# voletiv/mcvd-pytorch

Hardware: AMD Instinct MI355X
Metric: sampled frames/sec (whole node), SMMNIST 64x64 DDPM 100-step (higher is better)
Workload: dtype f32-equivalent: f32 storage and accumulation; 58 of 58 3x3 convs, 41 of 41 1x1 convs and the attention products (head dims 32..128) as SIX bf16 piece products of operands split EXACTLY into three bf16 pieces (all 24 bits, fp32 exponent range, less than one fp32 rounding per product; tests/test_gpu_p

## Files before the change

### mcvd_pytorch_amd/csrc/api.cpp

```cpp
#include <dlfcn.h>
#include <errno.h>
#include <fcntl.h>
#include <pthread.h>
#include <math.h>
#include <sys/file.h>
#include <sys/stat.h>
#include <unistd.h>
#include <stdio.h>
#include <stdlib.h>
#include <string.h>

#include <algorithm>
#include <cmath>
#include <mutex>
#include <new>
#include <vector>

#include "model.h"
#include "conv_kernels.h"
#include "inception.h"
#include "lpips.h"

using namespace mcvd;

// ... 298 lines not shown
    if (ok) { ctx->wino_selftest = 1; return 0; }
    ctx->wino_selftest = -1;
    ctx->bf16x3 = 0;
    ++ctx->epoch;
    set_error("self-test of the hand-scheduled Winograd kernels FAILED on this device (kernels that ran: %d %d %d; |bf16x3 - fp32 MFMA| = %.3e at "
              "scale %.3e; %zu values of the persistent form differ from the per-item form): the option bf16x3 was switched off for this context",
              ran[0], ran[1], ran[2], (double)d10, (double)scale, diff16);
    return MCVD_ESELFTEST;
    API_CATCH
}

int mcvd_ctx_clear_range(mcvd_ctx* ctx) {
    API_TRY
    MCVD_REQUIRE(ctx, "ctx is NULL");
    if (ctx->range_flag) MCVD_HIP_CHECK(hipMemsetAsync(ctx->range_flag, 0, sizeof(int), ctx->stream));
    return 0;
    API_CATCH
}

int mcvd_ctx_set_option(mcvd_ctx* ctx, const char* key, int value) {
    MCVD_REQUIRE(ctx && key, "ctx/key is NULL");
    ++ctx->epoch;
    if (!strcmp(key, "naive_conv")) ctx->naive_conv = value;
    else if (!strcmp(key, "naive_attn")) ctx->naive_attn = value;
    else if (!strcmp(key, "fir_form")) ctx->fir_form = value;
    else if (!strcmp(key, "dbg_skip_finalize")) ctx->dbg_skip_finalize = value;
    else if (!strcmp(key, "gn_producer")) ctx->gn_producer = value;
    else if (!strcmp(key, "graph")) ctx->graph = value;
    else if (!strcmp(key, "conv_shape")) ctx->conv_shape = value;
    else if (!strcmp(key, "conv_shape1")) ctx->conv_shape1 = value;
    else if (!strcmp(key, "profile")) ctx->profile = value;
    else if (!strcmp(key, "conv_wdma")) ctx->conv_wdma = value;
    else if (!strcmp(key, "autotune")) ctx->autotune = value;
    else if (!strcmp(key, "side_stream")) ctx->side_stream = value;
    else if (!strcmp(key, "share_fence")) ctx->share_fence = value;
    else if (!strcmp(key, "winograd")) ctx->winograd = value;
    else if (!strcmp(key, "conv_dma1")) ctx->conv_dma1 = value;
    else if (!strcmp(key, "bf16x3")) ctx->bf16x3 = value;
    else if (!strcmp(key, "f16x2")) {
        if (ctx->f16x2 != value) (void)mcvd_ctx_clear_range(ctx);
        ctx->f16x2 = value;
    }
    else if (!strcmp(key, "f16x1")) {
        if (ctx->f16x1 != value) (void)mcvd_ctx_clear_range(ctx);
        ctx->f16x1 = value;
    }
    else if (!strcmp(key, "conv_cot")) ctx->conv_cot = value;
    else if (!strcmp(key, "persist_grid")) ctx->persist_grid = value;
    else if (!strcmp(key, "temb_table")) ctx->temb_table = value;
    else if (!strcmp(key, "im2col_lds")) ctx->im2col_lds = value;
    else if (!strcmp(key, "gn_stats")) ctx->gn_stats = value;
    else if (!strcmp(key, "spade_fuse")) ctx->spade_fuse = value;
    else if (!strcmp(key, "attn_presplit")) ctx->attn_presplit = value;
    else {
        set_error("unknown option '%s'", key);
        return MCVD_EINVAL;
    }
    return 0;
}

static void default_schedule(mcvd_model* m) {
    const int T = m->d.num_classes;
    m->betas.assign(T, 0.f);
    m->alphas.assign(T, 0.f);
    m->alphas_prev.assign(T, 0.f);
    if (m->d.sigma_dist == 0) {
        const float start = m->d.sigma_begin, end = m->d.sigma_end;
        const float step = (end - start) / (float)(T - 1);
        for (int i = 0; i < T; ++i) m->betas[i] = (i < T / 2) ? start + step * (float)i : end - step * (float)(T - 1 - i);
        float p = 1.0f;
        for (int i = T - 1; i >= 0; --i) {
            p = p * (1.0f - m->betas[i]);
            m->alphas[i] = p;
        }
        for (int i = 0; i < T; ++i) m->alphas_prev[i] = (i + 1 < T) ? m->alphas[i + 1] : 1.0f;
    } else {
        std::vector<float> f(T + 1);
        const float s = 0.008f;
        for (int i = 0; i <= T; ++i) {
            const float t = (float)(T - i) / (float)T;
            const float c = cosf((t + s) / (1.0f + s) * (float)(M_PI / 2));
            f[i] = c * c;
        }
        for (int i = 0; i < T; ++i) m->alphas[i] = f[i] / f[T];
        for (int i = 0; i < T; ++i) m->alphas_prev[i] = (i + 1 < T) ? m->alphas[i + 1] : 1.0f;
        for (int i = 0; i < T; ++i) m->betas[i] = 1.0f - m->alphas[i] / m->alphas_prev[i];
    }
    const int half = m->d.ngf / 2;
    m->freqs.assign(half, 0.f);
    const float e = (float)(-(log(10000.0) / (double)(half - 1)));
    for (int k = 0; k < half; ++k) m->freqs[k] = expf((float)k * e);
}

int mcvd_model_create(mcvd_ctx* ctx, const mcvd_unet_desc* desc, mcvd_model** out) {
    API_TRY
    MCVD_REQUIRE(desc && out, "model_create: NULL argument");
    MCVD_REQUIRE(desc->sigma_dist == 0 || desc->sigma_dist == 1, "desc: sigma_dist=%d", desc->sigma_dist);
    mcvd_model* m = new mcvd_model();
    m->ctx = ctx;
    m->d = *desc;
    if (m->build_plan()) {
        delete m;
        return MCVD_EINVAL;
    }
    default_schedule(m);
    if (ctx) {
// ... 351 lines not shown
        kinds[i] = (int)op.kind;
        ks[i] = op.kind == OP_CONV ? op.ks : 0;
        ms[i] = t;
        const double HW = (double)op.H * op.W;
        const double cin = op.src0.C + (op.src1.kind == REF_NONE ? 0 : op.src1.C);
        double f = 0, by = 0;
        switch (op.kind) {
            case OP_CONV:
                f = 2.0 * B * HW * op.Cout * cin * op.ks * op.ks;
                by = 4.0 * (B * HW * (cin + op.Cout + (op.res.kind != REF_NONE ? op.Cout : 0)) + cin * op.ks * op.ks * op.Cout);
                break;
            case OP_GN: by = 4.0 * B * HW * cin; f = 4.0 * B * HW * cin; break;
            case OP_FIR: {
                const double o = op.up ? 4.0 : 0.25;
                by = 4.0 * B * HW * op.src0.C * (1.0 + o * (op.dst2.kind != REF_NONE ? 2.0 : 1.0));
                f = B * HW * op.src0.C * o * (op.up ? 8.0 : 32.0);
                break;
            }
            case OP_ATTN:
                f = 4.0 * B * HW * HW * op.Cout;
                by = 4.0 * B * HW * op.Cout * 4.0;
                break;
            case OP_APPLY: by = 4.0 * B * HW * cin * 4.0; f = 12.0 * B * HW * cin; break;
            case OP_TEMB: f = 2.0 * B * (m->d.ngf * m->T + (double)m->T * m->T); by = 4.0 * (m->d.ngf * m->T + (double)m->T * m->T); break;
            case OP_DENSE: f = 2.0 * B * m->T * m->NE; by = 4.0 * ((double)m->T * m->NE + B * m->NE); break;
            default: break;
        }
        flops[i] = f;
        bytes[i] = by;
    }
    return n;
}

int mcvd_model_op_info(mcvd_model* m, int i, int info[8]) {
    MCVD_REQUIRE(m && info && i >= 0 && i < (int)m->ops.size(), "op_info: index %d", i);
    const Op& op = m->ops[i];
    info[0] = (int)op.kind; info[1] = op.module; info[2] = op.ks; info[3] = op.H;
    info[4] = op.src0.C + (op.src1.kind == REF_NONE ? 0 : op.src1.C); info[5] = op.Cout;
    info[6] = op.res.kind != REF_NONE; info[7] = op.coef.kind != REF_NONE;
    if ((size_t)i < m->tuned_shape.size() && m->tuned_shape[i] >= 0) info[6] |= (m->tuned_shape[i] << 4) | (m->tuned_cot[i] << 8) | (1 << 12);
    return 0;
}

int mcvd_model_op_kernel(mcvd_model* m, int i) {
    if (!m || i < 0 || i >= (int)m->ops.size() || m->ops[i].kind != OP_CONV || (size_t)i >= m->ran_kernel.size()) return -1;
    return m->ran_kernel[i];
}

int mcvd_model_op_attention_kernel(mcvd_model* m, int i) {
    if (!m || i < 0 || i >= (int)m->ops.size() || m->ops[i].kind != OP_ATTN || (size_t)i >= m->ran_attn.size()) return -1;
    return m->ran_attn[i];
}

long mcvd_model_fused_launches(mcvd_model* m, int what) { return (m && what >= 0 && what < 4) ? m->fused_launches[what] : -1; }

int mcvd_model_module_output(mcvd_model* m, int module, int B, float* dst, int64_t capacity, int* C, int* H) {
    MCVD_REQUIRE(m && dst && B > 0 && B <= m->arena_B, "module_output: run a forward at batch >= B first");
    const Op* last = nullptr;
    for (const Op& op : m->ops)
        if (op.module == module && op.dst.kind == REF_ARENA) last = &op;
    MCVD_REQUIRE(last, "module_output: module %d has no workspace output", module);
    const int c = last->dst.C;
    int h = last->H;
    if (last->kind == OP_FIR) h = last->up ? 2 * h : h / 2;
    if (last->kind == OP_TEMB || last->kind == OP_DENSE) h = 0;
    const int64_t per = h ? (int64_t)c * h * h : c;
    MCVD_REQUIRE(per * B <= capacity, "module_output: capacity %lld < %lld", (long long)capacity, (long long)(per * B));
    MCVD_HIP_CHECK(hipMemcpyAsync(dst, m->arena + last->dst.off * (int64_t)B, (size_t)per * B * sizeof(float),
                                  hipMemcpyDeviceToDevice, m->ctx->stream));
    if (C) *C = c;
    if (H) *H = h;
    return 0;
}

struct GuidedCall {
    const float* cond_weak;
    float w;
    int weak_mask;
};

static int guided_begin(mcvd_model* m, const char* who, const float* cond, const GuidedCall& g, int B) {
    MCVD_REQUIRE(m->d.num_frames_cond > 0 && cond, "%s: guidance needs a net with conditioning frames (and its cond)", who);
    MCVD_REQUIRE(!m->d.noise_in_cond, "%s: guidance on a noise_in_cond net is not defined (two z per evaluation)", who);
    MCVD_REQUIRE(B <= (1 << 29), "%s: B = %d", who, B);
    if (int rc = m->prepare_B(2 * B)) return rc;
    if (int rc = m->ensure_guided(B, g.weak_mask)) return rc;
    const size_t cbytes = (size_t)B * m->d.channels * m->d.num_frames_cond * m->d.image_size * m->d.image_size * sizeof(float);
    hipStream_t s = m->ctx->stream;
    MCVD_HIP_CHECK(hipMemcpyAsync(m->gd_cond, cond, cbytes, hipMemcpyDeviceToDevice, s));
    char* weak = reinterpret_cast<char*>(m->gd_cond) + cbytes;
    if (g.cond_weak) MCVD_HIP_CHECK(hipMemcpyAsync(weak, g.cond_weak, cbytes, hipMemcpyDeviceToDevice, s));
    else MCVD_HIP_CHECK(hipMemsetAsync(weak, 0, cbytes, s));
    m->cond_cache_valid = false;
    return 0;
}

static int guided_dup_x(mcvd_model* m, const float* x, int64_t n) {
    hipStream_t s = m->ctx->stream;
    MCVD_HIP_CHECK(hipMemcpyAsync(m->gd_x, x, (size_t)n * sizeof(float), hipMemcpyDeviceToDevice, s));
    MCVD_HIP_CHECK(hipMemcpyAsync(m->gd_x + n, x, (size_t)n * sizeof(float), hipMemcpyDeviceToDevice, s));
    return 0;
}

static int sampler_run_impl(mcvd_model* m, int kind, float* x, const float* cond, const float* noise, uint64_t seed,
                            uint64_t sample_offset, int subsample_steps, int flags, double t_min, int B, const GuidedCall* g) {
    MCVD_REQUIRE(m && x && B > 0, "sampler_run: bad arguments");
    MCVD_REQUIRE(kind == MCVD_SAMPLER_DDPM || kind == MCVD_SAMPLER_DDIM, "sampler_run: kind %d", kind);
// ... 772 lines not shown
```

### mcvd_pytorch_amd/csrc/common.h

```cpp
#pragma once
#include <hip/hip_runtime.h>
#include <stdint.h>
#include <atomic>
#include <string>

#include "conv_kernels.h"


namespace mcvd {

__device__ __forceinline__ float fma_unpacked(float x, float a, float b) {
    float r;
    asm("v_fma_f32 %0, %1, %2, %3" : "=v"(r) : "v"(x), "v"(a), "v"(b));
    return r;
}

void set_error(const char* fmt, ...);
const char* get_error();

#define MCVD_HIP_CHECK(expr)                                                                  \
    do {                                                                                      \
        hipError_t _e = (expr);                                                               \
        if (_e != hipSuccess) {                                                               \
            mcvd::set_error("%s failed: %s (%s:%d)", #expr, hipGetErrorString(_e), __FILE__, __LINE__); \
// ... 15 lines not shown
        int dev = 0;
        if (hipGetDevice(&dev) != hipSuccess || dev < 0 || dev >= 64) return true;
        const unsigned long long bit = 1ull << dev;
        return (mask.load(std::memory_order_acquire) & bit) == 0;
    }
    void done() {
        int dev = 0;
        if (hipGetDevice(&dev) == hipSuccess && dev >= 0 && dev < 64) mask.fetch_or(1ull << dev, std::memory_order_release);
    }
};

static inline int ceil_div(int a, int b) { return (a + b - 1) / b; }
static inline int round_up(int a, int b) { return ceil_div(a, b) * b; }

struct GnOut {
    float* coef;
    int groups;
    float eps;
    int mode;
    const float* p0;
    const float* p1;
    int emb_stride, emb_off;
};

struct ConvArgs {
    const float* x0;
    const float* x1;
    int C0, C1;
    const float* coef;
    int act;
    const float* wp;
    const float* wpw;
    const float* wph;
    const float* wpb;
    const float* bias;
    const float* res;
    float out_scale;
    float* y;
    int B, Cin, CinP, Cout, CoutP, H, W;
    int ks;
    int cot;
    int shape_hint;
    int ksplit;
    float* part;
    size_t part_floats;
    int wdma;
    int pgrid;
    unsigned long long* dbg;
    float* stats;
    const float* gb;
    const float* coef2;
    float* kv_img;
    int kv_C, kv_D;
    int im2col;
    GnOut gno;
};
int last_conv_gn_fused();
void set_last_conv_gn_fused(int v);
bool ksplit_reduce_gn_usable(const ConvArgs& a);
int launch_ksplit_reduce_gn(const ConvArgs& a, hipStream_t s);
bool conv1x1_h2_kv_supported(const ConvArgs& a, int cot);
void set_last_conv_stats_np(int np);
int last_conv_stats_np();
int conv_cout_tile(int Cout);
int conv_chunk(int ks);
int launch_conv_mfma(const ConvArgs& a, hipStream_t s);
int launch_conv_naive(const ConvArgs& a, hipStream_t s);
int last_conv_kernel();
bool conv_kernel_usable(int id, const ConvArgs& a);
int conv_kernel_launch(int id, const ConvArgs& a, hipStream_t s);
int launch_im2col3x3(const float* x0, int C0, const float* x1, int C1, float* col, int B, int H, int W, int K, hipStream_t s);
int launch_taps_shift_add(const float* z, const float* bias, const float* res, float scale, float* y, int B, int Cout, int H, int W, hipStream_t s);
int launch_pack_conv_gemm_form(const float* w, float* wp, int Cout, int Cin, int form, int CoutP, hipStream_t s);
int conv_wino_require(ConvFamily family, const ConvArgs& a, const char* what);
dim3 wino_grid(const ConvArgs& a, bool g8, int bco, int parts);
int wino_launch_done(const ConvArgs& a, bool g8, int parts, hipStream_t s);
bool conv_wino_supported(int ks, int H, int W);
int conv_wino_cout_tile(int Cout);
int launch_conv_wino(const ConvArgs& a, hipStream_t s);
int launch_wino_ksplit_reduce(const ConvArgs& a, hipStream_t s);
int launch_conv_wino3(const ConvArgs& a, hipStream_t s);
long conv_wino3_weight_floats(int CinP, int CoutP);
int launch_conv_wino3p(const ConvArgs& a, hipStream_t s);
int launch_pack_wino3_weight(const float* w, float* wb, int Cout, int Cin, int CinP, int CoutP, hipStream_t s);
int launch_conv_wino2h(const ConvArgs& a, int np, hipStream_t s);
long conv_wino2h_weight_floats(int CinP, int CoutP);
int launch_pack_wino2h_weight(const float* w, float* wh, int Cout, int Cin, int CinP, int CoutP, hipStream_t s);
bool conv1x1_h2_supported(const ConvArgs& a, int cot, int np);
int launch_conv1x1_h2(const ConvArgs& a, int cot, hipStream_t s, int np);
long conv1x1_h2_weight_floats(int CinP, int CoutP, int np);
int launch_pack_conv1x1_h2(const float* wp, float* wh, int CinP, int CoutP, hipStream_t s, int np);
bool conv1x1_dma_supported(const ConvArgs& a, int ck, int pxw = 1);
int conv1x1_dma_cout_tile(int CoutP);
int launch_conv1x1_dma(const ConvArgs& a, int cot_req, int ck, hipStream_t s, int pxw = 1);
int launch_pack_wino_weight(const float* w, float* up, int Cout, int Cin, int CinP, int CoutP, hipStream_t s);
int launch_pack_conv_weight(const float* w, float* wp, int Cout, int Cin, int ks, int CinP, int CoutP, int nin,
                            int cout_off, hipStream_t s);

struct GnArgs {
    const float* x0;
    const float* x1;
    int C0, C1;
    int groups;
    float eps;
    int mode;
    const float* p0;
    const float* p1;
    int emb_stride, emb_off;
    float* coef;
    int B, HW;
};
int launch_gn_coef(const GnArgs& a, hipStream_t s);
int launch_gn_finalize(const GnArgs& a, const float* st0, int np0, const float* st1, int np1, hipStream_t s);

// ... 83 lines not shown
```

### mcvd_pytorch_amd/csrc/kernels/conv1x1_h2.cpp

```cpp
#include <stdlib.h>

#include "../common.h"
#include "pieces.h"

namespace mcvd {

typedef float f32x16 __attribute__((ext_vector_type(16)));
typedef float f32x2 __attribute__((ext_vector_type(2)));
typedef unsigned u32x4 __attribute__((ext_vector_type(4)));

__device__ __forceinline__ float silu_q(float v) { return v * __builtin_amdgcn_rcpf(1.0f + __expf(-v)); }

constexpr int Q1_PT = 128;
constexpr int Q1_CK = 16;
constexpr int Q1_NB = 4;
constexpr int Q1_MAXIMG = 4;

template <int NP, int COT, int PRO, int EXP = 0, bool KV = false, bool IM = false>
__global__ __launch_bounds__(256, 2) void conv1x1_h2_kernel(ConvArgs a, int ptiles, int nct) {
    typedef Pieces<NP> PX;
    constexpr int PT = Q1_PT, CK = Q1_CK, NB = Q1_NB, BCO = 32 * COT;
    constexpr int PPR = PT / 4;
    constexpr int RPS = 256 / PPR;
    constexpr int XSZ = CK * PT;
// ... 432 lines not shown
        if constexpr (NP == 3)
            MCVD_HIP_CHECK(hipFuncSetAttribute(reinterpret_cast<const void*>(&conv1x1_h2_kernel<3, COT, 1, 0, true>), hipFuncAttributeMaxDynamicSharedMemorySize, 160 * 1024));
        raised.done();
    }
#ifdef MCVD_DIAG
    {
        const char* es = getenv("MCVD_Q1_EXP");
        const int e = es ? atoi(es) : 0;
        if (e != 0 && NP == 3 && COT == 3) {
            static PerDeviceOnce raised2;
            if (raised2.first_use()) {
                (void)hipFuncSetAttribute(reinterpret_cast<const void*>(&conv1x1_h2_kernel<3, 3, 1, 1>), hipFuncAttributeMaxDynamicSharedMemorySize, 160 * 1024);
                (void)hipFuncSetAttribute(reinterpret_cast<const void*>(&conv1x1_h2_kernel<3, 3, 1, 2>), hipFuncAttributeMaxDynamicSharedMemorySize, 160 * 1024);
                (void)hipFuncSetAttribute(reinterpret_cast<const void*>(&conv1x1_h2_kernel<3, 3, 1, 4>), hipFuncAttributeMaxDynamicSharedMemorySize, 160 * 1024);
                (void)hipFuncSetAttribute(reinterpret_cast<const void*>(&conv1x1_h2_kernel<3, 3, 1, 6>), hipFuncAttributeMaxDynamicSharedMemorySize, 160 * 1024);
                (void)hipFuncSetAttribute(reinterpret_cast<const void*>(&conv1x1_h2_kernel<3, 3, 1, 7>), hipFuncAttributeMaxDynamicSharedMemorySize, 160 * 1024);
                (void)hipFuncSetAttribute(reinterpret_cast<const void*>(&conv1x1_h2_kernel<3, 3, 1, 15>), hipFuncAttributeMaxDynamicSharedMemorySize, 160 * 1024);
                (void)hipFuncSetAttribute(reinterpret_cast<const void*>(&conv1x1_h2_kernel<3, 3, 1, 16>), hipFuncAttributeMaxDynamicSharedMemorySize, 160 * 1024);
                raised2.done();
            }
            switch (e) {
                case 1: hipLaunchKernelGGL((conv1x1_h2_kernel<3, 3, 1, 1>), grid, dim3(256), lds, s, a, ptiles, nct); break;
                case 2: hipLaunchKernelGGL((conv1x1_h2_kernel<3, 3, 1, 2>), grid, dim3(256), lds, s, a, ptiles, nct); break;
                case 4: hipLaunchKernelGGL((conv1x1_h2_kernel<3, 3, 1, 4>), grid, dim3(256), lds, s, a, ptiles, nct); break;
                case 6: hipLaunchKernelGGL((conv1x1_h2_kernel<3, 3, 1, 6>), grid, dim3(256), lds, s, a, ptiles, nct); break;
                case 7: hipLaunchKernelGGL((conv1x1_h2_kernel<3, 3, 1, 7>), grid, dim3(256), lds, s, a, ptiles, nct); break;
                case 16: hipLaunchKernelGGL((conv1x1_h2_kernel<3, 3, 1, 16>), grid, dim3(256), lds, s, a, ptiles, nct); break;
                default: hipLaunchKernelGGL((conv1x1_h2_kernel<3, 3, 1, 15>), grid, dim3(256), lds, s, a, ptiles, nct); break;
            }
            MCVD_HIP_CHECK(hipGetLastError());
            return 0;
        }
    }
    if constexpr (NP == 3) {
        static const bool noprio = getenv("MCVD_Q1_NOPRIO") && atoi(getenv("MCVD_Q1_NOPRIO")) != 0;
        if (noprio) {
            static PerDeviceOnce raised3;
            if (raised3.first_use()) {
                (void)hipFuncSetAttribute(reinterpret_cast<const void*>(&conv1x1_h2_kernel<NP, COT, 0, 16>), hipFuncAttributeMaxDynamicSharedMemorySize, 160 * 1024);
                (void)hipFuncSetAttribute(reinterpret_cast<const void*>(&conv1x1_h2_kernel<NP, COT, 1, 16>), hipFuncAttributeMaxDynamicSharedMemorySize, 160 * 1024);
                (void)hipFuncSetAttribute(reinterpret_cast<const void*>(&conv1x1_h2_kernel<NP, COT, 2, 16>), hipFuncAttributeMaxDynamicSharedMemorySize, 160 * 1024);
                raised3.done();
            }
            if (!a.coef) hipLaunchKernelGGL((conv1x1_h2_kernel<NP, COT, 0, 16>), grid, dim3(256), lds, s, a, ptiles, nct);
            else if (!a.act) hipLaunchKernelGGL((conv1x1_h2_kernel<NP, COT, 1, 16>), grid, dim3(256), lds, s, a, ptiles, nct);
            else hipLaunchKernelGGL((conv1x1_h2_kernel<NP, COT, 2, 16>), grid, dim3(256), lds, s, a, ptiles, nct);
            MCVD_HIP_CHECK(hipGetLastError());
            return 0;
        }
    }
#endif
    if constexpr (NP == 3) {
        if (a.kv_img && a.coef && !a.act) {
            hipLaunchKernelGGL((conv1x1_h2_kernel<3, COT, 1, 0, true>), grid, dim3(256), lds, s, a, ptiles, nct);
            MCVD_HIP_CHECK(hipGetLastError());
            return 0;
        }
    }
    if (!a.coef)
        hipLaunchKernelGGL((conv1x1_h2_kernel<NP, COT, 0>), grid, dim3(256), lds, s, a, ptiles, nct);
    else if (!a.act)
        hipLaunchKernelGGL((conv1x1_h2_kernel<NP, COT, 1>), grid, dim3(256), lds, s, a, ptiles, nct);
    else
        hipLaunchKernelGGL((conv1x1_h2_kernel<NP, COT, 2>), grid, dim3(256), lds, s, a, ptiles, nct);
    MCVD_HIP_CHECK(hipGetLastError());
    return 0;
}

template <int NP>
static int q1_launch_cot(const ConvArgs& a, int cot, hipStream_t s) {
    switch (cot) {
        case 1: return q1_launch<NP, 1>(a, s);
        case 2: return q1_launch<NP, 2>(a, s);
        case 3: return q1_launch<NP, 3>(a, s);
        default: return q1_launch<NP, 4>(a, s);
    }
}

bool conv1x1_h2_kv_supported(const ConvArgs& a, int cot) {
    return a.kv_img && a.kv_C > 0 && a.Cout == 3 * a.kv_C && a.kv_D % 32 == 0 && a.kv_C % a.kv_D == 0 && a.coef && !a.act && !a.res && a.out_scale == 1.0f &&
           !a.stats && conv1x1_h2_supported(a, cot, 3);
}

int launch_conv1x1_h2(const ConvArgs& a, int cot, hipStream_t s, int np) {
    MCVD_REQUIRE(!a.kv_img || (np == 3 && conv1x1_h2_kv_supported(a, cot)), "conv1x1 split-operand GEMM: K / V piece images requested for a launch that cannot write them");
    MCVD_REQUIRE(conv1x1_h2_supported(a, cot, np), "conv1x1 split-operand GEMM: unsupported (np=%d ks=%d H=%d W=%d Cin=%d C0=%d cot=%d, weight pieces %s)",
                 np, a.ks, a.H, a.W, a.Cin, a.C0, cot, (np == 2 ? a.wph : a.wpb) ? "present" : "missing");
    const int rc = np == 2 ? q1_launch_cot<2>(a, cot, s) : q1_launch_cot<3>(a, cot, s);
    const int HW = a.H * a.W;
    if (rc == 0 && a.stats && (HW >= Q1_PT || HW == 64)) set_last_conv_stats_np(HW >= Q1_PT ? HW / Q1_PT : 1);
    return rc;
}

__global__ void q1_absmax_kernel(const float* w, long n, unsigned* hdr) {
    float m = 0.0f;
    for (long i = blockIdx.x * (long)blockDim.x + threadIdx.x; i < n; i += (long)gridDim.x * blockDim.x) m = fmaxf(m, fabsf(w[i]));
#pragma unroll
    for (int o = 32; o > 0; o >>= 1) m = fmaxf(m, __shfl_xor(m, o));
    if ((threadIdx.x & 63) == 0) atomicMax(hdr, __float_as_uint(m));
}

__global__ void pack_conv1x1_h2_kernel(const float* wp, float* wh, int CinP, int CoutP) {
    const float wmax = wh[0];
    int k = 0;
    (void)frexpf(wmax, &k);
    const int e = (wmax > 0.0f && wmax < 3.0e38f) ? min(max(14 - k, -60), 60) : 0;
    const float scale = ldexpf(1.0f, e);
    if (blockIdx.x == 0 && threadIdx.x == 0) { wh[1] = scale; wh[2] = ldexpf(1.0f, -e); }
    _Float16* dst = reinterpret_cast<_Float16*>(wh + Pieces<2>::HDR);
    const long n = (long)CinP * CoutP;
    const int NS = CoutP / 32;
    for (long i = blockIdx.x * (long)blockDim.x + threadIdx.x; i < n; i += (long)gridDim.x * blockDim.x) {
        const int co = (int)(i % CoutP), ci = (int)(i / CoutP);
        const float us = wp[i] * scale;
        const _Float16 h1 = (_Float16)us;
        const _Float16 h2 = (_Float16)(us - (float)h1);
        const int cc = ci & 15, h = cc & 1, el = cc >> 1, lane = h * 32 + (co & 31);
        const long o = (((long)(ci >> 4) * NS + (co >> 5)) * 2) * 512 + (lane * 4 + (el >> 1)) * 2 + (el & 1);
        dst[o] = h1;
        dst[o + 512] = h2;
    }
}

__global__ void pack_conv1x1_b3_kernel(const float* wp, unsigned short* dst, int CinP, int CoutP) {
    const long n = (long)CinP * CoutP;
    const int NS = CoutP / 32;
    for (long i = blockIdx.x * (long)blockDim.x + threadIdx.x; i < n; i += (long)gridDim.x * blockDim.x) {
        const int co = (int)(i % CoutP), ci = (int)(i / CoutP);
        const float u = wp[i];
        const unsigned short h1 = px_bf16_rne(u);
        const float r1 = u - px_bf16_f32(h1);
        const unsigned short h2 = px_bf16_rne(r1);
        const float r2 = r1 - px_bf16_f32(h2);
        const unsigned short h3 = px_bf16_rne(r2);
        const int cc = ci & 15, h = cc & 1, el = cc >> 1, lane = h * 32 + (co & 31);
        const long o = (((long)(ci >> 4) * NS + (co >> 5)) * 3) * 512 + (lane * 4 + (el >> 1)) * 2 + (el & 1);
        dst[o] = h1;
        dst[o + 512] = h2;
        dst[o + 1024] = h3;
    }
// ... 22 lines not shown
```

### mcvd_pytorch_amd/csrc/model.cpp

```cpp
#include "model.h"
#include "conv_kernels.h"

#include <math.h>
#include <stdarg.h>
#include <stdio.h>
#include <string.h>

#include <algorithm>
#include <tuple>

namespace mcvd {

static thread_local char g_err[1024] = "";
void set_error(const char* fmt, ...) {
    va_list ap;
    va_start(ap, fmt);
    vsnprintf(g_err, sizeof(g_err), fmt, ap);
    va_end(ap);
}
const char* get_error() { return g_err; }

static int gn_groups(int ch) {
    int g = std::min(ch / 4, 32);
    while (g > 1 && ch % g != 0) --g;
// ... 749 lines not shown
        const int np = pieces(a.shape_hint);
        for (int c = 4; c >= 1 && !conv1x1_h2_supported(a, a.cot, np); --c)
            if (conv1x1_h2_supported(a, c, np)) a.cot = c;
    }
    if (!(a.shape_hint < 0 && tuned_B == a.B && oi < tuned_shape.size() && tuned_shape[oi] >= 0)) return;
    a.shape_hint = tuned_shape[oi];
    a.cot = tuned_cot[oi];
    const bool raw_in = conv_input_raw(op);
    if (!ctx->f16x1 || raw_in) a.shape_hint = without_f16x1(a.shape_hint);
    if ((!ctx->f16x2 || raw_in) && without_f16x2(a.shape_hint) != a.shape_hint) {
        a.shape_hint = without_f16x2(a.shape_hint);
        if (conv_kernel(a.shape_hint).own_cot && !conv_kernel_usable(a.shape_hint, a)) a.cot = op.cot;
    }
    if (!ctx->bf16x3 && without_bf16x3(a.shape_hint) != a.shape_hint) {
        a.shape_hint = without_bf16x3(a.shape_hint);
        a.cot = op.cot;
    }
}

int mcvd_model::apply_spade(const Op& op, const Io& io, ConvArgs& a) {
    if (a.shape_hint == CK_RETIRED_SPADE_WINO || a.shape_hint == CK_RETIRED_SPADE_WINO_K2) a.shape_hint = CK_AUTO;
    const bool want_fused = ctx->spade_fuse && !ctx->naive_conv && ctx->winograd;
    ConvArgs t = a;
    t.shape_hint = a.shape_hint == CK_WINO_K2 ? CK_WINO_K2 : CK_WINO;
    t.ksplit = k_parts(t.shape_hint);
    bool fused = want_fused && conv_kernel_usable(CK_WINO, t);
    if (!fused && t.ksplit == 2) { t.ksplit = 0; t.shape_hint = CK_WINO; fused = want_fused && conv_kernel_usable(CK_WINO, t); }
    if (fused) {
        a.shape_hint = t.shape_hint;
        ++fused_launches[2];
        return 0;
    }
    float* tmp = resolve(op.tmp, io);
    if (int rc = launch_spade_apply(a.x0, a.C0, a.x1, a.C1, a.coef, a.gb, a.coef2, tmp, a.B, op.H * op.W, op_stream ? op_stream : ctx->stream)) return rc;
    read_materialised(a, tmp);
    return 0;
}

void mcvd_model::set_gn_producer(const Op& op, const Io& io, ConvArgs& a) {
    gn_done[op.gn_next] = 0;
    if (ctx->gn_producer && ctx->gn_stats && a.stats && op.ks == 3 && !ctx->dbg_skip_finalize) gn_params(a.gno, ops[op.gn_next], io);
}

void mcvd_model::set_kv_presplit(const Op& op, const Io& io, ConvArgs& a) {
    kv_live[op.attn_op] = 0;
    const Op& at = ops[op.attn_op];
    const bool want = ctx->attn_presplit && !ctx->naive_conv && ctx->bf16x3 && !ctx->f16x2 && (ctx->naive_attn == 0 || ctx->naive_attn == 4) &&
                      !(ctx->share_fence && mcvd_ctx_shares_device(ctx)) && attn_h2p_supported(at.Cout, at.heads, at.H * at.W) && a.shape_hint == CK_GEMM1_BF16X3;
    if (!want) return;
    ConvArgs t = a;
    t.kv_img = resolve(op.kv, io);
    t.kv_C = at.Cout;
    t.kv_D = at.Cout / at.heads;
    if (conv1x1_h2_kv_supported(t, t.cot)) {
        a = t;
        kv_live[op.attn_op] = 1;
    }
}

int mcvd_model::launch_conv_op(const Op& op, const Io& io) {
    hipStream_t s = op_stream ? op_stream : ctx->stream;
    const size_t oi = (size_t)(&op - ops.data());
    ConvArgs a = conv_args(op, io, true);
    MCVD_REQUIRE(a.x0 && (a.C1 == 0 || a.x1), "forward: module %d needs a conditioning tensor (cond is NULL)", op.module);
    select_hint(op, a);
    if (op.gb.kind != REF_NONE)
        if (int rc = apply_spade(op, io, a)) return rc;
    a.stats = (ctx->gn_stats && op.stats.kind != REF_NONE && !ctx->naive_conv && (op.ks == 3 || ctx->gn_stats >= 2 || conv_kernel(a.shape_hint).family == CF_SPLIT1))
                  ? resolve(op.stats, io) : nullptr;
    if (ran_kernel.size() != ops.size()) ran_kernel.assign(ops.size(), -1);
    if (kv_live.size() != ops.size()) kv_live.assign(ops.size(), 0);
    if (gn_done.size() != ops.size()) gn_done.assign(ops.size(), 0);
    if (op.gn_next >= 0) set_gn_producer(op, io, a);
    if (op.attn_op >= 0) set_kv_presplit(op, io, a);
    if (ctx->naive_conv) {
        stats_np[oi] = 0;
        ran_kernel[oi] = -2;
        return launch_conv_naive(a, s);
    }
    if (conv_kernel(a.shape_hint).family == CF_GEMM3) {
        if (gemm_form_usable(op, a)) {
            const int rc = launch_gemm_form(op, a, resolve(op.alt_buf, io), s);
            stats_np[oi] = a.stats ? last_conv_stats_np() : 0;
            ran_kernel[oi] = op.alt_kind;
            return rc;
        }
        a.shape_hint = CK_AUTO;
        a.cot = op.cot;
    }
    const int rc = launch_conv_mfma(a, s);
    stats_np[oi] = a.stats ? last_conv_stats_np() : 0;
    ran_kernel[oi] = last_conv_kernel();
    if (rc == 0 && a.gno.coef && last_conv_gn_fused()) {
        gn_done[op.gn_next] = 1;
        ++fused_launches[3];
    }
    return rc;
}

int mcvd_model::launch_op(const Op& op, const float* x, const void* lab, const float* cond, float* out, int B) {
    hipStream_t s = op_stream ? op_stream : ctx->stream;
    const Io io{x, cond, out, B};
    auto at = [&](const TRef& r) { return resolve(r, io); };
    switch (op.kind) {
        case OP_TEMB: {
            if (temb_row_live) return 0;
            const float* w0 = blob + params[find_param("unet.all_modules.0.weight")].off;
            const float* b0 = blob + params[find_param("unet.all_modules.0.bias")].off;
            const float* w1 = blob + params[find_param("unet.all_modules.1.weight")].off;
            const float* b1 = blob + params[find_param("unet.all_modules.1.bias")].off;
            const float* emb = d.cond_emb ? blob + params[find_param("unet.all_modules.2.weight")].off : nullptr;
            return launch_temb_mlp(lab, labels_f32, packed + freqs_off, w0, b0, w1, b1, at(op.dst), one_temb_row() ? 1 : B, d.ngf, T, emb, cond_mask, s);
        }
        case OP_DENSE:
            if (temb_row_live) return 0;
            return launch_dense_all(at(op.src0), packed + dense_wt, packed + dense_bias, at(op.dst), one_temb_row() ? 1 : B, T, NE, s);
        case OP_GN:
            return launch_gn(op, io);
        case OP_CONV:
            return launch_conv_op(op, io);
        case OP_FIR: {
            const float* gb = at(op.gb);
            return launch_fir2(at(op.src0), at(op.coef), op.act, op.up, at(op.dst), B, op.src0.C, op.H, op.W, gb,
                               gb ? gb + (size_t)op.src0.C * op.H * op.W : nullptr, at(op.coef2), at(op.dst2), s, ctx->fir_form);
        }
        case OP_NEAREST:
            MCVD_REQUIRE(cond, "forward: SPADE model needs the conditioning tensor");
            return launch_nearest_resize(at(op.src0), at(op.dst), B * op.src0.C, d.image_size, d.image_size, op.H, op.W, s);
        case OP_CONDNOISE: {
            MCVD_REQUIRE(cond, "forward: noise_in_cond model needs the conditioning tensor");
            MCVD_REQUIRE(!labels_f32, "forward: noise_in_cond indexes alphas with the labels; float timesteps are not valid there");
            const int64_t per = (int64_t)op.src0.C * d.image_size * d.image_size;
            if (!alphas_dev) MCVD_HIP_CHECK(hipMalloc((void**)&alphas_dev, (size_t)d.num_classes * sizeof(float)));
            if (!alphas_dev_valid) {
                MCVD_HIP_CHECK(hipMemcpyAsync(alphas_dev, alphas.data(), (size_t)d.num_classes * sizeof(float), hipMemcpyHostToDevice, s));
                alphas_dev_valid = true;
            }
            const float* z = cond_noise_src;
            if (z) {
                cond_noise_src += per * B;
            } else {
                if (cond_gamma_k > 0.0f) {
                    if (int rc = launch_gamma_noise(cond_z, nullptr, cond_gamma_k, cond_gamma_theta, cond_gamma_kt, cond_gamma_sd,
                                                    cond_noise_seed, cond_noise_offset, (1ull << 32) + cond_noise_draw, B, per, s))
                        return rc;
// ... 366 lines not shown
```

### mcvd_pytorch_amd/csrc/model.h

```cpp
#pragma once
#include <atomic>
#include <map>
#include <string>
#include <vector>

#include "../../include/mcvd_hip.h"
#include "common.h"
#include "conv_tuner.h"

struct mcvd_ctx {
    int device = 0;
    int shared_device = 0;
    hipStream_t stream = nullptr;
    int naive_conv = 0;
    int naive_attn = 0;
    int gn_producer = 1;
    int dbg_skip_finalize = 0;
    int fir_form = 0;
    int graph = 0;
    hipStream_t cap = nullptr;
    std::atomic<unsigned> epoch{0};
    int conv_shape = -1;
    int conv_shape1 = -1;
    int winograd = 1;
    int persist_grid = 0;
    int temb_table = 1;
    int im2col_lds = 1;
    int wino_selftest = 0;
    int conv_cot = 0;
    int bf16x3 = 1;
    int f16x2 = 0;
    int f16x1 = 0;
    int conv_dma1 = 1;
    int conv_wdma = 1;
    int share_fence = 0;
    int side_stream = 0;
    hipStream_t side = nullptr;
    hipEvent_t ev_fork = nullptr, ev_join = nullptr;
    int spade_fuse = 0;
    int attn_presplit = 1;
    int gn_stats = 1;
    int autotune = 1;
    int profile = 0;
    unsigned long long* dbg = nullptr;
    const float* spade_gb = nullptr;
    const float* spade_coef2 = nullptr;
    float* stats_buf = nullptr;
    int* range_flag = nullptr;
    float* scratch = nullptr;
    size_t scratch_bytes = 0;
    int ensure_scratch(size_t bytes);
};

bool mcvd_ctx_shares_device(const mcvd_ctx* c);

namespace mcvd {

struct ParamInfo {
    std::string name;
    int64_t shape[4] = {0, 0, 0, 0};
    int ndim = 0;
    int64_t off = 0;
    int64_t numel = 0;
    bool set = false;
};

enum RefKind { REF_NONE = 0, REF_ARENA, REF_X, REF_COND, REF_OUT };
struct TRef {
    RefKind kind = REF_NONE;
    int64_t off = 0;
    int C = 0;
};

enum OpKind { OP_TEMB, OP_DENSE, OP_GN, OP_CONV, OP_FIR, OP_ATTN, OP_NEAREST, OP_COEF2, OP_APPLY, OP_CONDNOISE };

struct Op {
    OpKind kind;
    int module = -1;
    TRef src0, src1, dst, res;
    int H = 0, W = 0;
    int Cout = 0, ks = 0;
    int groups = 0;
    float eps = 0.f;
    int gn_mode = 0;
    int64_t p0 = -1, p1 = -1;
    int emb_off = 0;
    TRef coef;
    int act = 0;
    int64_t wp = -1, bias = -1;
    int64_t wpw = -1;
    int64_t wph = -1;
    int64_t wpb = -1;
    int CinP = 0, CoutP = 0, cot = 0;
// ... 54 lines not shown
    float* blob = nullptr;

    std::vector<mcvd::Op> ops;
    std::vector<mcvd::DenseEntry> dense;
    std::vector<mcvd::ConvPack> packs;
    int64_t packed_floats = 0;
    float* packed = nullptr;
    long long* coef2_desc_dev = nullptr;
    int coef2_first = -1, coef2_count = 0, coef2_cmax = 0;
    float* packed_h = nullptr;
    int64_t packed_h_floats = 0;
    bool packed_h_valid = false;
    int ensure_f16x2_weights();
    int64_t dense_wt = -1, dense_bias = -1, freqs_off = -1;
    int NE = 0;
    int T = 0;
    int first_module = 2;
    mcvd::TRef cond_src;
    const int32_t* cond_mask = nullptr;
    float* alphas_dev = nullptr;
    bool alphas_dev_valid = false;
    float* cond_z = nullptr;
    const float* cond_noise_src = nullptr;
    uint64_t cond_noise_seed = 0, cond_noise_offset = 0, cond_noise_draw = 0;
    float cond_gamma_kt = 0.f, cond_gamma_sd = 1.f;
    float* noise_buf = nullptr;
    float cond_gamma_k = 0.f, cond_gamma_theta = 0.f;
    std::vector<float> k_cum, theta_t;
    float* gamma_dev = nullptr;
    bool gamma_dev_valid = false;
    float* dsm_buf = nullptr;
    int dsm_B = 0;

    int64_t arena_per_sample = 0;
    float* arena = nullptr;
    int arena_B = 0;
    int64_t* labels = nullptr;
    float* eps_buf = nullptr;
    float* labels_f = nullptr;
    float* fp_buf = nullptr;
    int fp_B = 0;
    float* gd_x = nullptr;
    float* gd_cond = nullptr;
    int32_t* gd_mask = nullptr;
    int gd_B = 0, gd_mask_B = 0, gd_mask_val = -1;
    int ensure_guided(int B, int weak_mask);
    float* ksplit_buf = nullptr;
    size_t ksplit_floats = 0;

    std::vector<float> betas, alphas, alphas_prev, freqs;

    std::vector<int> stats_np;
    std::vector<signed char> kv_live;
    long fused_launches[4] = {0, 0, 0, 0};
    std::vector<signed char> gn_done;
    std::vector<int> ran_kernel;
    std::vector<int> ran_attn;
    std::vector<int> tuned_shape, tuned_cot;
    int tuned_B = 0;
    int tuned_sig = -1;
    std::map<int, std::pair<std::vector<int>, std::vector<int>>> tuned_cache;
    int autotune(int B);
    void sync_tuning_options();
    mcvd::TunerOptions tuner_options() const;
    mcvd::TunerLayer tuner_layer(const mcvd::Op& op, int B) const;

    std::vector<hipEvent_t> ev;
    bool profile_armed = false;
    int profile_B = 0;

    const float* prepared_cond = nullptr;
    int prepared_B = 0;
    bool cond_cache_valid = false;
    bool has_prep = false;
    int prepare_B(int B);
    int run_prep(const float* cond, int B);
    int prepare_cond(const float* cond, int B);

    struct GraphKey {
        const float* x = nullptr; const void* lab = nullptr; const float* cond = nullptr; float* out = nullptr;
        const void* mask = nullptr;
        int B = 0, labels_f32 = 0; unsigned epoch = 0, ctx_epoch = 0;
        bool operator==(const GraphKey& o) const {
            return x == o.x && lab == o.lab && cond == o.cond && out == o.out && mask == o.mask && B == o.B &&
                   labels_f32 == o.labels_f32 && epoch == o.epoch && ctx_epoch == o.ctx_epoch;
        }
    };
    GraphKey graph_key, graph_seen;
    hipGraphExec_t graph_exec = nullptr;
    unsigned epoch = 0;
    long graph_replays = 0, graph_captures = 0;
    void drop_graph();
    int forward_ops(const float* x, const void* labels, const float* cond, float* out, int B);

    hipStream_t op_stream = nullptr;
    int build_plan();
    int add_param(const std::string& name, std::initializer_list<int64_t> shape);
    int find_param(const char* name) const;
    int ensure_workspace(int B);
    int ensure_ksplit(int B);
    float* temb_tab = nullptr;
    float* temb_tmp = nullptr;
    int64_t* temb_lab = nullptr;
    size_t temb_rows_cap = 0;
    int temb_row_live = 0;
    int profile_temb_skipped = 0;
    int prepare_temb_table(const std::vector<int>& labels);
// ... 22 lines not shown
```

Before: 260.5.

## Add pixel-stationary split-operand QKV 1x1 conv kernel with LDS-resident activation pieces

Adds a new kernel for the attention q|k|v 1x1 projection. Each block splits a 64-pixel activation tile (with the per-channel affine coefficient applied) into bf16 pieces once and keeps them in LDS. Waves then stream weight pieces for many 32-channel output slices against that tile, writing Q directly and K/V as presplit piece images. The intent is to stop re-reading and re-splitting activations for every output tile, and the new path is on by default through a new option. The cost is a large dynamic LDS allocation (up to 160KB), which limits occupancy, and a grid-sizing heuristic tuned to 256 CUs.

```diff
diff --git a/mcvd_pytorch_amd/csrc/api.cpp b/mcvd_pytorch_amd/csrc/api.cpp
--- a/mcvd_pytorch_amd/csrc/api.cpp
+++ b/mcvd_pytorch_amd/csrc/api.cpp
@@ -374,6 +374,7 @@
     else if (!strcmp(key, "gn_stats")) ctx->gn_stats = value;
     else if (!strcmp(key, "spade_fuse")) ctx->spade_fuse = value;
     else if (!strcmp(key, "attn_presplit")) ctx->attn_presplit = value;
+    else if (!strcmp(key, "qkv_stationary")) ctx->qkv_stationary = value;
     else {
         set_error("unknown option '%s'", key);
         return MCVD_EINVAL;
@@ -831,7 +832,7 @@
     return m->ran_attn[i];
 }
 
-long mcvd_model_fused_launches(mcvd_model* m, int what) { return (m && what >= 0 && what < 4) ? m->fused_launches[what] : -1; }
+long mcvd_model_fused_launches(mcvd_model* m, int what) { return (m && what >= 0 && what < 5) ? m->fused_launches[what] : -1; }
 
 int mcvd_model_module_output(mcvd_model* m, int module, int B, float* dst, int64_t capacity, int* C, int* H) {
     MCVD_REQUIRE(m && dst && B > 0 && B <= m->arena_B, "module_output: run a forward at batch >= B first");
diff --git a/mcvd_pytorch_amd/csrc/common.h b/mcvd_pytorch_amd/csrc/common.h
--- a/mcvd_pytorch_amd/csrc/common.h
+++ b/mcvd_pytorch_amd/csrc/common.h
@@ -91,6 +91,7 @@
     const float* coef2;
     float* kv_img;
     int kv_C, kv_D;
+    int kv_stationary;
     int im2col;
     GnOut gno;
 };
@@ -99,6 +100,10 @@
 bool ksplit_reduce_gn_usable(const ConvArgs& a);
 int launch_ksplit_reduce_gn(const ConvArgs& a, hipStream_t s);
 bool conv1x1_h2_kv_supported(const ConvArgs& a, int cot);
+bool conv1x1_h2s_admits(const ConvArgs& a);
+int launch_conv1x1_h2s(const ConvArgs& a, hipStream_t s);
+int last_conv_qkv_stationary();
+void set_last_conv_qkv_stationary(int v);
 void set_last_conv_stats_np(int np);
 int last_conv_stats_np();
 int conv_cout_tile(int Cout);
diff --git a/mcvd_pytorch_amd/csrc/kernels/conv1x1_h2.cpp b/mcvd_pytorch_amd/csrc/kernels/conv1x1_h2.cpp
--- a/mcvd_pytorch_amd/csrc/kernels/conv1x1_h2.cpp
+++ b/mcvd_pytorch_amd/csrc/kernels/conv1x1_h2.cpp
@@ -508,6 +508,10 @@
 #endif
     if constexpr (NP == 3) {
         if (a.kv_img && a.coef && !a.act) {
+            if (a.kv_stationary && conv1x1_h2s_admits(a)) {
+                set_last_conv_qkv_stationary(1);
+                return launch_conv1x1_h2s(a, s);
+            }
             hipLaunchKernelGGL((conv1x1_h2_kernel<3, COT, 1, 0, true>), grid, dim3(256), lds, s, a, ptiles, nct);
             MCVD_HIP_CHECK(hipGetLastError());
             return 0;
@@ -542,6 +546,7 @@
     MCVD_REQUIRE(!a.kv_img || (np == 3 && conv1x1_h2_kv_supported(a, cot)), "conv1x1 split-operand GEMM: K / V piece images requested for a launch that cannot write them");
     MCVD_REQUIRE(conv1x1_h2_supported(a, cot, np), "conv1x1 split-operand GEMM: unsupported (np=%d ks=%d H=%d W=%d Cin=%d C0=%d cot=%d, weight pieces %s)",
                  np, a.ks, a.H, a.W, a.Cin, a.C0, cot, (np == 2 ? a.wph : a.wpb) ? "present" : "missing");
+    set_last_conv_qkv_stationary(0);
     const int rc = np == 2 ? q1_launch_cot<2>(a, cot, s) : q1_launch_cot<3>(a, cot, s);
     const int HW = a.H * a.W;
     if (rc == 0 && a.stats && (HW >= Q1_PT || HW == 64)) set_last_conv_stats_np(HW >= Q1_PT ? HW / Q1_PT : 1);
diff --git a/mcvd_pytorch_amd/csrc/kernels/conv1x1_h2s.cpp b/mcvd_pytorch_amd/csrc/kernels/conv1x1_h2s.cpp
--- /dev/null
+++ b/mcvd_pytorch_amd/csrc/kernels/conv1x1_h2s.cpp
@@ -0,0 +1,232 @@
+#include "../common.h"
+#include "pieces.h"
+
+namespace mcvd {
+
+typedef float f32x16 __attribute__((ext_vector_type(16)));
+typedef float f32x4 __attribute__((ext_vector_type(4)));
+typedef float f32x2 __attribute__((ext_vector_type(2)));
+typedef unsigned u32x4 __attribute__((ext_vector_type(4)));
+
+constexpr int S1_PT = 64;
+constexpr int S1_CK = 16;
+constexpr int S1_WAVES = 8;
+constexpr int S1_PITCH = 36;
+constexpr int S1_SLICE = 32 * S1_PITCH;
+constexpr int S1_CUS = 256;
+constexpr size_t S1_LDS_MAX = 160 * 1024;
+
+static size_t s1_lds_bytes(int Cin) { return (size_t)Cin * (S1_PT * 3 * 2) + (size_t)S1_WAVES * S1_SLICE * sizeof(float); }
+
+__global__ __launch_bounds__(S1_WAVES * 64) void conv1x1_h2s_kernel(ConvArgs a, int tiles, int ng, int upg, int nunits) {
+    typedef Pieces<3> PX;
+    extern __shared__ __attribute__((aligned(16))) float smem[];
+    const int tid = threadIdx.x, lane = tid & 63, l31 = lane & 31, half = lane >> 5;
+    const int wave = __builtin_amdgcn_readfirstlane(tid >> 6);
+    const int Cin = a.Cin, nchunks = Cin / S1_CK, HW = a.H * a.W, NS = a.CoutP / 32;
+    u32x4* sB = reinterpret_cast<u32x4*>(smem);
+    float* sO = smem + nchunks * (2 * 3 * 256) + wave * S1_SLICE;
+
+    int tile, grp;
+    if (tiles < 8) {
+        tile = blockIdx.x % tiles;
+        grp = blockIdx.x / tiles;
+    } else {
+        const int xcd = blockIdx.x & 7, slot = blockIdx.x >> 3;
+        tile = (slot / ng) * 8 + xcd;
+        grp = slot - (slot / ng) * ng;
+    }
+    if (tile >= tiles || grp >= ng) return;
+    const int b = (int)(((long)tile * S1_PT) / HW), p0 = (int)((long)tile * S1_PT - (long)b * HW);
+
+    {
+        const float* xb = a.x0 + (long)b * a.C0 * HW + p0 + l31;
+        const float* cb = a.coef + (long)b * Cin * 2;
+        const int nitems = nchunks * 2;
+        for (int it = wave; it < nitems; it += 2 * S1_WAVES) {
+            float bv[2][8];
+            f32x2 cf[2][8];
+#pragma unroll
+            for (int u = 0; u < 2; ++u) {
+                const int item = it + u * S1_WAVES;
+                if (item < nitems) {
+                    const int c0 = (item >> 1) * S1_CK + half;
+                    const float* xs = xb + (long)c0 * HW + (item & 1) * 32;
+#pragma unroll
+                    for (int e = 0; e < 8; ++e) {
+                        bv[u][e] = xs[(long)(2 * e) * HW];
+                        cf[u][e] = *reinterpret_cast<const f32x2*>(cb + (c0 + 2 * e) * 2);
+                    }
+                }
+            }
+#pragma unroll
+            for (int u = 0; u < 2; ++u) {
+                const int item = it + u * S1_WAVES;
+                if (item < nitems) {
+#pragma unroll
+                    for (int e = 0; e < 8; ++e)
+                        asm("v_fma_f32 %0, %1, %2, %3" : "=v"(bv[u][e]) : "v"(bv[u][e]), "v"(cf[u][e].x), "v"(cf[u][e].y));
+                    unsigned w[4][3];
+#pragma unroll
+                    for (int j = 0; j < 4; ++j) PX::split<false>(bv[u][2 * j], bv[u][2 * j + 1], w[j]);
+#pragma unroll
+                    for (int p = 0; p < 3; ++p) sB[(item * 3 + p) * 64 + lane] = u32x4{w[0][p], w[1][p], w[2][p], w[3][p]};
+                }
+            }
+        }
+    }
+    __syncthreads();
+
+    const int lo = grp * upg, hi = min(lo + upg, nunits);
+    const u32x4* wq = reinterpret_cast<const u32x4*>(a.wpb) + lane;
+    const int Cq = a.kv_C, D = a.kv_D, DT = D >> 5, heads = Cq / D, ntl = HW >> 5;
+    unsigned* img = reinterpret_cast<unsigned*>(a.kv_img);
+#define S1_LOADA(SET, st, c)                                                        \
+    {                                                                               \
+        const u32x4* w_ = wq + ((long)(c) * NS + (st)) * (3 * 64);                  \
+        SET[0] = w_[0]; SET[1] = w_[64]; SET[2] = w_[128];                          \
+    }
+#define S1_READB(SET, c)                                                            \
+    {                                                                               \
+        const u32x4* b_ = sB + (c) * (2 * 3 * 64) + lane;                           \
+        _Pragma("unroll") for (int q = 0; q < 6; ++q) SET[q] = b_[q * 64];          \
+    }
+#define S1_MMA(AC, BC)                                                              \
+    _Pragma("unroll") for (int k = 0; k < PX::NPROD; ++k)                           \
+        _Pragma("unroll") for (int t = 0; t < 2; ++t) acc[t] = PX::mfma(AC[PX::PA(k)], BC[t * 3 + PX::PB(k)], acc[t]);
+#define S1_STEP(AC, BC, AN2, BN1, c)                                                \
+    {                                                                               \
+        S1_LOADA(AN2, st, min((c) + 2, nchunks - 1))                                \
+        S1_READB(BN1, min((c) + 1, nchunks - 1))                                    \
+        __builtin_amdgcn_sched_barrier(0);       \
+        S1_MMA(AC, BC)                                                              \
+        __builtin_amdgcn_sched_barrier(0);                                          \
+    }
+    u32x4 A0[3], A1[3], A2[3], B0[6], B1[6], B2[6];
+    if (lo + wave < hi) {
+        S1_LOADA(A0, lo + wave, 0)
+        S1_LOADA(A1, lo + wave, min(1, nchunks - 1))
+    }
+    for (int st = lo + wave; st < hi; st += S1_WAVES) {
+        f32x16 acc[2];
+#pragma unroll
+        for (int t = 0; t < 2; ++t)
+#pragma unroll
+            for (int r = 0; r < 16; ++r) acc[t][r] = 0.0f;
+        S1_READB(B0, 0)
+        int c = 0;
+        for (; c + 3 <= nchunks; c += 3) {
+            S1_STEP(A0, B0, A2, B1, c)
+            S1_STEP(A1, B1, A0, B2, c + 1)
+            S1_STEP(A2, B2, A1, B0, c + 2)
+        }
+        if (c < nchunks) {
+            S1_READB(B1, min(c + 1, nchunks - 1))
+            S1_MMA(A0, B0)
+            if (c + 1 < nchunks) S1_MMA(A1, B1)
+        }
+        {
+            const int stn = st + S1_WAVES < hi ? st + S1_WAVES : st;
+            S1_LOADA(A0, stn, 0)
+            S1_LOADA(A1, stn, min(1, nchunks - 1))
+        }
+
+        const int cs = st * 32;
+        const int which = cs / Cq;
+        const int within = cs - which * Cq, head = within / D, ch0 = within - head * D;
+#pragma unroll
+        for (int t = 0; t < 2; ++t) {
+            const int pix0 = p0 + t * 32;
+            asm volatile("s_waitcnt lgkmcnt(0)" ::: "memory");
+#pragma unroll
+            for (int r = 0; r < 16; ++r) sO[((r & 3) + 8 * (r >> 2) + 4 * half) * S1_PITCH + l31] = acc[t][r];
+            asm volatile("s_waitcnt lgkmcnt(0)" ::: "memory");
+            if (which == 0) {
+                const int px4 = lane & 7, cr = lane >> 3;
+#pragma unroll
+                for (int k = 0; k < 4; ++k) {
+                    const int cl = cr + 8 * k, co = cs + cl;
+                    f32x4 v = *reinterpret_cast<const f32x4*>(sO + cl * S1_PITCH + px4 * 4);
+                    v = (v + a.bias[co] + 0.0f) * a.out_scale;
+                    *reinterpret_cast<f32x4*>(a.y + ((long)b * a.Cout + co) * HW + pix0 + px4 * 4) = v;
+                }
+            } else if (which == 1) {
+#pragma unroll
+                for (int rnd = 0; rnd < 2; ++rnd) {
+                    const int item = rnd * 64 + lane;
+                    const int rp = item >> 3, p4 = item & 7;
+                    const int st_l = rp >> 3, j = (rp >> 1) & 3, h = rp & 1;
+                    const int rl = 16 * st_l + 4 * j + h;
+                    const int pix = pix0 + p4 * 4;
+                    const f32x4 v0 = *reinterpret_cast<const f32x4*>(sO + rl * S1_PITCH + p4 * 4) + a.bias[cs + rl];
+                    const f32x4 v1 = *reinterpret_cast<const f32x4*>(sO + (rl + 2) * S1_PITCH + p4 * 4) + a.bias[cs + rl + 2];
+                    unsigned w[4][3];
+#pragma unroll
+                    for (int i4 = 0; i4 < 4; ++i4) PX::split<false>(v0[i4], v1[i4], w[i4]);
+                    const int stq = (ch0 >> 4) + st_l;
+                    unsigned* d1 = img + ((long)(b * heads + head) * ntl + (pix >> 5)) * (3072 * DT) + (stq * 3 * 4 + j) * 64 + h * 32 + (pix & 31);
+#pragma unroll
+                    for (int pc = 0; pc < 3; ++pc) *reinterpret_cast<u32x4*>(d1 + pc * 256) = u32x4{w[0][pc], w[1][pc], w[2][pc], w[3][pc]};
+                }
+            } else {
+#pragma unroll
+                for (int rnd = 0; rnd < 2; ++rnd) {
+                    const int item = rnd * 64 + lane;
+                    const int m = item & 31, g2 = item >> 5;
+                    const int s2 = (g2 >> 1) & 1, h = g2 & 1;
+                    const int kb = 16 * s2 + 4 * h;
+                    const float bs = a.bias[cs + m];
+                    const f32x4 v0 = *reinterpret_cast<const f32x4*>(sO + m * S1_PITCH + kb) + bs;
+                    const f32x4 v1 = *reinterpret_cast<const f32x4*>(sO + m * S1_PITCH + kb + 8) + bs;
+                    unsigned wa[3], wb[3], wc[3], wd[3];
+                    PX::split<false>(v0[0], v0[1], wa);
+                    PX::split<false>(v0[2], v0[3], wb);
+                    PX::split<false>(v1[0], v1[1], wc);
+                    PX::split<false>(v1[2], v1[3], wd);
+                    unsigned* d1 = img + ((long)(b * heads + head) * ntl + (pix0 >> 5)) * (3072 * DT) + 1536 * DT +
+                                   ((((ch0 >> 5) * 2 + s2) * 3) * 64 + h * 32 + m) * 4;
+#pragma unroll
+                    for (int pc = 0; pc < 3; ++pc) *reinterpret_cast<u32x4*>(d1 + pc * 256) = u32x4{wa[pc], wb[pc], wc[pc], wd[pc]};
+                }
+            }
+        }
+    }
+#undef S1_STEP
+#undef S1_MMA
+#undef S1_READB
+#undef S1_LOADA
+}
+
+bool conv1x1_h2s_admits(const ConvArgs& a) {
+    const int HW = a.H * a.W;
+    return a.kv_img && a.coef && !a.act && a.C1 == 0 && a.C0 == a.Cin && a.wpb && a.ks == 1 && !a.im2col && HW % S1_PT == 0 &&
+           a.Cin % S1_CK == 0 && a.Cin <= a.CinP && a.CoutP % 32 == 0 && a.Cout % 32 == 0 && a.Cout <= a.CoutP &&
+           (long)a.B * a.Cin * HW < (1L << 31) && s1_lds_bytes(a.Cin) <= S1_LDS_MAX;
+}
+
+static thread_local int g_last_stationary = 0;
+int last_conv_qkv_stationary() { return g_last_stationary; }
+void set_last_conv_qkv_stationary(int v) { g_last_stationary = v; }
+
+int launch_conv1x1_h2s(const ConvArgs& a, hipStream_t s) {
+    MCVD_REQUIRE(conv1x1_h2s_admits(a), "conv1x1 pixel-stationary q|k|v GEMM: unsupported (H=%d W=%d Cin=%d C1=%d Cout=%d)", a.H, a.W, a.Cin, a.C1, a.Cout);
+    const int tiles = (int)((long)a.B * a.H * a.W / S1_PT);
+    const int nunits = a.Cout / 32;
+    int ng = (S1_CUS + tiles - 1) / tiles;
+    if (ng > nunits / S1_WAVES) ng = nunits / S1_WAVES;
+    if (ng < 1) ng = 1;
+    const int upg = (nunits + ng - 1) / ng;
+    ng = (nunits + upg - 1) / upg;
+    const size_t lds = s1_lds_bytes(a.Cin);
+    static PerDeviceOnce raised;
+    if (raised.first_use()) {
+        MCVD_HIP_CHECK(hipFuncSetAttribute(reinterpret_cast<const void*>(&conv1x1_h2s_kernel), hipFuncAttributeMaxDynamicSharedMemorySize, (int)S1_LDS_MAX));
+        raised.done();
+    }
+    const dim3 grid(tiles < 8 ? tiles * ng : ((tiles + 7) / 8) * 8 * ng);
+    hipLaunchKernelGGL(conv1x1_h2s_kernel, grid, dim3(S1_WAVES * 64), lds, s, a, tiles, ng, upg, nunits);
+    MCVD_HIP_CHECK(hipGetLastError());
+    return 0;
+}
+
+}
diff --git a/mcvd_pytorch_amd/csrc/model.cpp b/mcvd_pytorch_amd/csrc/model.cpp
--- a/mcvd_pytorch_amd/csrc/model.cpp
+++ b/mcvd_pytorch_amd/csrc/model.cpp
@@ -825,6 +825,7 @@
     t.kv_img = resolve(op.kv, io);
     t.kv_C = at.Cout;
     t.kv_D = at.Cout / at.heads;
+    t.kv_stationary = ctx->qkv_stationary != 0;
     if (conv1x1_h2_kv_supported(t, t.cot)) {
         a = t;
         kv_live[op.attn_op] = 1;
@@ -861,9 +862,11 @@
         a.shape_hint = CK_AUTO;
         a.cot = op.cot;
     }
+    set_last_conv_qkv_stationary(0);
     const int rc = launch_conv_mfma(a, s);
     stats_np[oi] = a.stats ? last_conv_stats_np() : 0;
     ran_kernel[oi] = last_conv_kernel();
+    if (rc == 0 && a.kv_img && last_conv_qkv_stationary()) ++fused_launches[4];
     if (rc == 0 && a.gno.coef && last_conv_gn_fused()) {
         gn_done[op.gn_next] = 1;
         ++fused_launches[3];
diff --git a/mcvd_pytorch_amd/csrc/model.h b/mcvd_pytorch_amd/csrc/model.h
--- a/mcvd_pytorch_amd/csrc/model.h
+++ b/mcvd_pytorch_amd/csrc/model.h
@@ -39,6 +39,7 @@
     hipEvent_t ev_fork = nullptr, ev_join = nullptr;
     int spade_fuse = 0;
     int attn_presplit = 1;
+    int qkv_stationary = 1;
     int gn_stats = 1;
     int autotune = 1;
     int profile = 0;
@@ -199,7 +200,7 @@
 
     std::vector<int> stats_np;
     std::vector<signed char> kv_live;
-    long fused_launches[4] = {0, 0, 0, 0};
+    long fused_launches[5] = {0, 0, 0, 0, 0};
     std::vector<signed char> gn_done;
     std::vector<int> ran_kernel;
     std::vector<int> ran_attn;
```

Result: no change. 262.0 (median of 6 runs) (+0.6%).
